# lyclyc52/NeRF_RPN

Measured on AMD Instinct MI355X. Metric: scenes/sec (160^3x4 grids, VGG19-3D+FPN+RPN fwd+bwd), higher is better.
Workload: dtype bf16; 1 GPU; configs[1]: one 160x160x160x4 rgb-sigma grid per GPU, VGG19-EF 3D + FPN + anchor RPN (OBB, 16 GT boxes per scene), fwd+bwd+clip+AdamW, random-init weights; scenes_per_gpu=1, parallelism=dp1, world_size_seen=1, backend=single process

## Files before the change

include/nerfrpn.h:

```cpp
#ifndef NERFRPN_H
#define NERFRPN_H

#include <stddef.h>
#include <stdint.h>

#ifdef __cplusplus
extern "C" {
#endif

typedef void *nrpn_stream_t;

enum nrpn_status {
  NRPN_OK = 0,
  NRPN_ERR_ARG = -1,
  NRPN_ERR_LAUNCH = -2,
  NRPN_ERR_DEVICE = -3
};

enum nrpn_dtype { NRPN_F32 = 0, NRPN_BF16 = 1 };

const char *nrpn_last_error(void);
int nrpn_abi_version(void);
int nrpn_check_device(int ordinal);

// ... 44 lines not shown
                         const int32_t *d_count, int64_t n, int box_dim, int post_top_n, float *out_boxes,
                         float *out_scores, float *out_levels, int32_t *d_out_count, nrpn_stream_t stream);

int nrpn_match_anchors_f32(const int32_t *table, int64_t total_anchors, const float *gt_aabb, int num_gt,
                           float fg_thresh, float bg_thresh, const float *h_ori_size3, float *labels,
                           int32_t *matched, float *workspace, nrpn_stream_t stream);
int nrpn_obb_to_aabb_f32(const float *obb, float *aabb, int64_t n, nrpn_stream_t stream);

size_t nrpn_sample_workspace_bytes(void);
int nrpn_sample_pos_neg(const float *labels, int64_t total, int max_pos, int batch, int64_t seed, void *workspace, int64_t *out_pos,
                        int64_t *out_neg, int32_t *counts, nrpn_stream_t stream);
int nrpn_rpn_sampled_loss_f32(const float *logits, const float *deltas, int dw, const float *targets,
                              const int64_t *pos, int64_t npos, const int64_t *neg, int64_t nneg, float beta,
                              float *loss2, float *g_logits, float *g_deltas, nrpn_stream_t stream);

enum { NRPN_CONV_BIAS = 1, NRPN_CONV_RELU = 2, NRPN_CONV_OUT_F32 = 4,
       NRPN_CONV_DEBUG_ALIAS_TAPS = 256, NRPN_CONV_DEBUG_NO_SYNC = 512,
       NRPN_CONV_DEBUG_STAGGER = 1024,
       NRPN_CONV_DEBUG_VARIANT = 0x3000 };
int nrpn_pack_conv_weight(const float *w_ref, int cout, int cin, int taps, int dtype, void *wp_fwd, void *wp_dgrad,
                          int rows_total, int row_offset, nrpn_stream_t stream);
int nrpn_unpack_conv_wgrad(const float *gw_packed, int cout, int cin, int taps, int rows_total, int row_offset,
                           float *gw_ref, int accumulate, int slices, nrpn_stream_t stream);
size_t nrpn_conv3d_fwd_workspace_bytes(int n, int gx, int gy, int gz, int cin, int cout, int ksize, int dtype);
int nrpn_conv3d_fwd(const void *x, const void *wp, const float *bias, void *y, int n, int gx, int gy, int gz, int cin,
                    int cout, int wrows, int ksize, int dtype, int flags, void *workspace, const void *relu_mask,
                    nrpn_stream_t stream);
enum { NRPN_TILE_AUTO = 0, NRPN_TILE_128 = 128, NRPN_TILE_256X128_WS = 256, NRPN_TILE_256X256 = 512, NRPN_TILE_256X256_W4 = 1024,
       NRPN_TILE_HALO = 2048  };
typedef struct nrpn_conv_opts {
  int32_t size;
  int32_t tile;
  int32_t lds_dma;
  int32_t kstep_bytes;
  int32_t stagger;
  int32_t big_split;
  int32_t debug;
  int32_t halo_pairing;
  const float *scale;
  const void *relu_mask;
  float *stats;
} nrpn_conv_opts;
int nrpn_conv3d_fwd_ex(const void *x, const void *wp, const float *bias, void *y, int n, int gx, int gy, int gz, int cin,
                       int cout, int wrows, int ksize, int dtype, int flags, void *workspace, const nrpn_conv_opts *opts,
                       nrpn_stream_t stream);
size_t nrpn_conv3d_fwd_workspace_bytes_ex(int n, int gx, int gy, int gz, int cin, int cout, int ksize, int dtype,
                                          const nrpn_conv_opts *opts);
int nrpn_conv3d_fwd_plan_ex(int n, int gx, int gy, int gz, int cin, int cout, int ksize, int dtype, const nrpn_conv_opts *opts);
int nrpn_conv3d_fwd_stats_rows_ex(int n, int gx, int gy, int gz, int cin, int cout, int ksize, int dtype, const nrpn_conv_opts *opts);
size_t nrpn_conv3d_wgrad_workspace_bytes(int n, int gx, int gy, int gz, int cin, int cout, int wrows, int ksize, int dtype);
int nrpn_conv3d_wgrad_slices(int n, int gx, int gy, int gz, int cin, int cout, int wrows, int ksize, int dtype);
enum { NRPN_WGRAD_ACC_BIAS = 1, NRPN_WGRAD_MASK_READY = 2,
       NRPN_WGRAD_DEFER_BIAS = 4  };
int nrpn_conv3d_wgrad(const void *x, const void *dy, float *gw_packed, float *gbias, int n, int gx, int gy, int gz,
                      int cin, int cout, int wrows, int ksize, int dtype, int accumulate_bias, void *workspace,
                      nrpn_stream_t stream);
int nrpn_conv3d_fwd_ragged(const void *x, const void *wp, const float *bias, void *y, int nseg, const int32_t *dims, int cin,
                           int cout, int wrows, int ksize, int dtype, int flags, void *workspace, nrpn_stream_t stream);
int nrpn_conv3d_wgrad_ragged(const void *x, const void *dy, float *gw_packed, float *gbias, int nseg, const int32_t *dims,
                             int cin, int cout, int wrows, int ksize, int dtype, int accumulate_bias, void *workspace,
                             nrpn_stream_t stream);
size_t nrpn_cone_workspace_bytes(int64_t total_voxels);
int nrpn_cone_build(const int64_t *pos, const int64_t *neg, const int32_t *counts, int n_scenes, int64_t pos_stride, int64_t neg_stride,
                    int nlevels, const int64_t *level_anchor_off, int num_anchors, const int32_t *dims, int depth, uint32_t *lists,
                    int64_t cap, int32_t *counts_out, void *workspace, nrpn_stream_t stream);
size_t nrpn_conv3d_fwd_rows_workspace_bytes(int64_t nrows, int cin, int cout, int ksize, int dtype);
int nrpn_conv3d_fwd_rows(const void *x, const void *wp, const float *bias, void *y, const uint32_t *rows, int64_t nrows, int nseg,
                         const int32_t *dims, int cin, int cout, int wrows, int ksize, int dtype, int flags, const void *relu_mask,
                         void *workspace, nrpn_stream_t stream);
int nrpn_conv3d_wgrad_rows(const void *x, const void *dy, float *gw_packed, float *gbias, const uint32_t *rows, int64_t nrows, int nseg,
                           const int32_t *dims, int cin, int cout, int wrows, int ksize, int dtype, int accumulate_bias, void *workspace,
                           nrpn_stream_t stream);
int nrpn_conv3d_fwd_plan(int n, int gx, int gy, int gz, int cin, int cout, int ksize, int dtype);
int nrpn_conv3d_fwd_stats_rows(int n, int gx, int gy, int gz, int cin, int cout, int ksize, int dtype);
int nrpn_conv3d_fwd_stats(const void *x, const void *wp, const float *bias, void *y, int n, int gx, int gy, int gz, int cin,
                          int cout, int wrows, int ksize, int dtype, int flags, float *stats, nrpn_stream_t stream);
int nrpn_bn_stats_finalize(const float *partials, int nparts, int64_t rows, int c, float *mean, float *var, float *running_mean,
                           float *running_var, float momentum, nrpn_stream_t stream);
int nrpn_conv3d_wgrad_plan(int n, int gx, int gy, int gz, int cin, int cout, int wrows, int ksize, int dtype);
int nrpn_stem_kpad(int dtype);
int nrpn_pack_stem_weight(const float *w_ref, int cout, int dtype, void *wp, nrpn_stream_t stream);
int nrpn_stem_wgrad_slices(int n, int gx, int gy, int gz, int cout, int stride, int dtype);
int64_t nrpn_stem_wgrad_slice_floats(int n, int gx, int gy, int gz, int cout, int stride, int dtype);
int nrpn_unpack_stem_wgrad(const float *gw_packed, int cout, int dtype, float *gw_ref, int accumulate, int slices,
                           int64_t slice_floats, nrpn_stream_t stream);
int nrpn_conv3d_stem_fwd(const void *x, const void *wp, const float *bias, void *y, int n, int gx, int gy, int gz,
                         int cout, int stride, int dtype, int flags, nrpn_stream_t stream);
int nrpn_stem_halo_supported(int gz, int cout, int stride, int dtype);
int nrpn_stem_halo_kpad(void);
int nrpn_pack_stem_weight_halo(const float *w_ref, int cout, void *wp, nrpn_stream_t stream);
int nrpn_conv3d_stem_fwd_halo(const void *x, const void *wp, const float *bias, const float *scale, void *y, int n, int gx, int gy,
                              int gz, int cout, int flags, nrpn_stream_t stream);
int nrpn_conv3d_stem_fwd_ex(const void *x, const void *wp, const float *bias, void *y, int n, int gx, int gy, int gz,
                            int cout, int stride, int dtype, int flags, const nrpn_conv_opts *opts, nrpn_stream_t stream);
size_t nrpn_stem_wgrad_workspace_bytes(int n, int gx, int gy, int gz, int cout, int stride, int dtype);
int nrpn_conv3d_stem_wgrad(const void *x, const void *dy, float *gw_packed, float *gbias, int n, int gx, int gy, int gz,
                           int cout, int stride, int dtype, int accumulate_bias, void *workspace, nrpn_stream_t stream);

size_t nrpn_bn_workspace_bytes(int64_t rows, int c);
int nrpn_bn_stats(const void *x, int64_t rows, int c, int dtype, float *mean, float *var, float *running_mean,
                  float *running_var, float momentum, void *workspace, nrpn_stream_t stream);
int nrpn_bn_apply(const void *x, void *y, int64_t rows, int c, int dtype, const float *mean, const float *var,
                  const float *gamma, const float *beta, float eps, int relu, nrpn_stream_t stream);
int nrpn_bn_backward(const void *x, const void *y, const void *dy, void *dx, int64_t rows, int c, int dtype,
                     const float *mean, const float *var, const float *gamma, const float *beta, float eps, int relu,
                     float *dgamma, float *dbeta, float *acc_dgamma, float *acc_dbeta, void *workspace, nrpn_stream_t stream);
int nrpn_relu_backward(const void *y, const void *dy, void *dx, int64_t count, int dtype, nrpn_stream_t stream);
int nrpn_pool_out_size(int in, int k, int s, int p, int ceil_mode);
int nrpn_maxpool3d_fwd(const void *x, void *y, int8_t *argmax, int n, int gx, int gy, int gz, int c, int k, int s,
                       int p, int ceil_mode, int dtype, nrpn_stream_t stream);
int nrpn_maxpool3d_bwd(const void *dy, const int8_t *argmax, void *dx, int n, int gx, int gy, int gz, int c, int k,
                       int s, int p, int ceil_mode, int dtype, nrpn_stream_t stream);
int nrpn_upsample_add_fwd(void *fine, const void *coarse, int n, int fx, int fy, int fz, int cx, int cy, int cz, int c,
                          int dtype, nrpn_stream_t stream);
int nrpn_upsample_add_bwd(const void *dfine, void *dcoarse, int n, int fx, int fy, int fz, int cx, int cy, int cz,
                          int c, int dtype, int accumulate, nrpn_stream_t stream);
int nrpn_subsample3d(const void *src, void *dst, int n, int gx, int gy, int gz, int c, int stride, int backward, int dtype,
                     nrpn_stream_t stream);
int nrpn_add_relu(const void *a, const void *b, void *y, int64_t count, int relu, int dtype, nrpn_stream_t stream);
int nrpn_ingest_rgbsigma(const void *src, int src_is_u8, void *dst, int64_t voxels, int alpha_mode, int dtype, nrpn_stream_t stream);
int nrpn_ingest_augment(const void *src, int src_is_u8, void *dst, int w, int l, int h, int alpha_mode, int dtype, int rot90,
                        int z_up, int flip0, int flip1, const float *h_xform, nrpn_stream_t stream);
int nrpn_ncdhw_to_ndhwc(const float *src, void *dst, int n, int c, int64_t voxels, int dtype, nrpn_stream_t stream);
int nrpn_ndhwc_to_ncdhw(const void *src, float *dst, int n, int c, int64_t voxels, int dtype, nrpn_stream_t stream);
int nrpn_cast(const void *src, void *dst, int64_t count, int src_dtype, int dst_dtype, nrpn_stream_t stream);
size_t nrpn_column_sum_workspace_bytes(int64_t rows, int c);
int nrpn_column_sum_f32(const float *x, int64_t rows, int c, float *out, int accumulate, void *workspace, nrpn_stream_t stream);
int nrpn_split_bf16x3(const float *src, int64_t rows, int c, void *interleaved, int ipattern, void *planes, int nplanes, int ppattern,
                      nrpn_stream_t stream);

int nrpn_patchify(const void *x, void *y, int n, int gx, int gy, int gz, int patch, int dtype, nrpn_stream_t stream);
int nrpn_layernorm_fwd(const void *x, void *y, const float *gamma, const float *beta, float *mean, float *rstd, int64_t rows,
                       int c, float eps, int dtype, nrpn_stream_t stream);
size_t nrpn_layernorm_workspace_bytes(int64_t rows, int c);
int nrpn_layernorm_bwd(const void *x, const void *dy, void *dx, const float *gamma, const float *mean, const float *rstd,
                       float *dgamma, float *dbeta, int64_t rows, int c, int dtype, int accumulate_params, void *workspace,
                       nrpn_stream_t stream);
int nrpn_gelu(const void *x, const void *dy, void *out, int64_t count, int backward, int dtype, nrpn_stream_t stream);
int nrpn_scale_add(const void *a, const void *b, const float *scale, void *y, int n, int64_t per_sample, int dtype,
                   nrpn_stream_t stream);
int nrpn_patch_merge(const void *src, void *dst, int n, int gx, int gy, int gz, int c, int backward, int dtype,
                     nrpn_stream_t stream);
int nrpn_window_attn_fwd(const void *qkv, const float *qkv_bias, const float *bias_table, const int32_t *rel_index, void *out,
                         int n, int gx, int gy, int gz, int c, int heads, int shift, int dtype, nrpn_stream_t stream);
size_t nrpn_window_attn_bwd_workspace_bytes(int n, int gx, int gy, int gz, int heads);
int nrpn_window_attn_bwd(const void *qkv, const float *qkv_bias, const float *bias_table, const int32_t *rel_index,
                         const void *dout, void *dqkv, float *dtable, float *dbias_pad, int n, int gx, int gy, int gz, int c,
                         int heads, int shift, int dtype, int accumulate_table, void *workspace, nrpn_stream_t stream);

size_t nrpn_groupnorm_workspace_bytes(int n, int c, int groups);
int nrpn_groupnorm_fwd(const void *x, void *y, const float *gamma, const float *beta, float *mean, float *rstd, int n,
                       int64_t rows, int c, int groups, float eps, int relu, int dtype, void *workspace, nrpn_stream_t stream);
int nrpn_groupnorm_bwd(const void *x, const void *y, const void *dy, void *dx, const float *gamma, const float *mean,
                       const float *rstd, float *dgamma, float *dbeta, int n, int64_t rows, int c, int groups, int relu, int dtype,
                       int accumulate_params, void *workspace, nrpn_stream_t stream);
int nrpn_fcos_reduce_floats(void);
int nrpn_fcos_head_out_f32(const float *cls_out, const float *box_out, int wrows, const float *scale, float stride_mul,
                           int norm_reg, int reg_dim, int ctr_on_reg, int64_t rows, float *logits, float *reg, float *ctr,
                           nrpn_stream_t stream);
int nrpn_fcos_head_out_bwd_f32(const float *box_out, int wrows, const float *scale, float stride_mul, int norm_reg, int reg_dim,
                               int ctr_on_reg, int64_t rows, const float *d_logits, const float *d_reg, const float *d_ctr,
                               float *d_cls_out, float *d_box_out, float *d_scale, nrpn_stream_t stream);
int nrpn_fcos_gt_summary_f32(const float *gt, int count, int width, float *summary, nrpn_stream_t stream);
int nrpn_fcos_targets_f32(const float *summary, const int32_t *gt_offsets, int n, int levels, const int32_t *dims,
                          const int32_t *strides, const float *ori_sizes, float radius, int norm_reg, int reg_dim, int8_t *labels,
                          float *reg_targets, int32_t *num_pos, nrpn_stream_t stream);
// ... 148 lines not shown
```

include/nerfrpn_tools.h:

```cpp
#ifndef NERFRPN_TOOLS_H
#define NERFRPN_TOOLS_H
#include "nerfrpn.h"

#ifdef __cplusplus
extern "C" {
#endif

int nrpn_set_conv_kstep_bytes(int kb);
int nrpn_set_conv_lds_dma(int on);
int nrpn_set_conv_tile_m(int bm);
int nrpn_set_conv_halo_auto(int on);
int nrpn_set_conv_halo_pairing(int mode);
int nrpn_set_conv_stagger(int on);
int nrpn_set_conv_big_split(int on);
int nrpn_set_wgrad_big_tile(int on);
int nrpn_set_wgrad_pack2(int on);
int nrpn_set_sumsq_form(int form, int grid);
int nrpn_set_wgrad_transpose_read(int on);
int nrpn_set_rows_big_tile(int on);
int nrpn_set_rows_tail_split(int on);
int nrpn_set_bn_fast(int on);
int nrpn_set_bn_reduce_v8(int on);
int nrpn_set_pool_fast(int on);
int nrpn_set_gn_fast(int on);
int64_t nrpn_fastdiv_host(int64_t n, int64_t d);
int nrpn_set_window_attn_mfma(int on);

#ifdef __cplusplus
}
#endif
#endif
```

nerf_rpn_amd/csrc/conv3d.hip:

```cpp
#include "conv_common.cuh"
#include "conv_plan.h"

#ifndef NRPN_HALO_PAIRING_DEFAULT
#define NRPN_HALO_PAIRING_DEFAULT 2
#endif

template <typename T, int BN, int MODE, bool OUTF32, int KB, bool GLDS, int BM = 128, bool ROWS = false>
__global__ void __launch_bounds__(256, BM == 128 ? 2 : 1) conv_igemm_kernel(const ConvArgs p) {
  constexpr int WAVES_N = (BN == 128) ? 2 : 1;
  constexpr int TM = BM / (32 * (4 / WAVES_N));
  constexpr int TN = 2;
  constexpr int KE = KB / (int)sizeof(T);
  constexpr int PPR = KB / 16;
  constexpr int RSTEP = 256 / PPR;
  constexpr int A_RPT = BM / RSTEP;
  constexpr int B_RPT = BN / RSTEP;
  constexpr int SWZ_SH = (KB == 64) ? 2 : 1;
  constexpr int A_BYTES = BM * KB, B_BYTES = BN * KB;
  extern __shared__ __attribute__((aligned(16))) char lds[];

  const int tid = threadIdx.x, lane = tid & 63, wave = tid >> 6;
  const int wm = wave / WAVES_N, wn = wave % WAVES_N;
  const unsigned ntiles = (p.Cout + BN - 1) / BN;
  const unsigned tiles = (unsigned)((p.M + BM - 1) / BM) * ntiles;
// ... 2480 lines not shown
  return wgrad_plan(conv_shape(n, gx, gy, gz, cin, cout, wrows, ksize, dtype), cin, 0, wg_knobs());
}
extern "C" size_t nrpn_conv3d_wgrad_bias_offset(int n, int gx, int gy, int gz, int ksize) {
  return wgrad_mask_bytes((long long)n * gx * gy * gz, ksize == 3 ? 27 : 1);
}
extern "C" size_t nrpn_conv3d_wgrad_workspace_bytes(int n, int gx, int gy, int gz, int cin, int cout, int wrows, int ksize, int dtype) {
  const WgPlan pl = wgrad_query(n, gx, gy, gz, cin, cout, wrows, ksize, dtype);
  return pl.bias_off + pl.bias_bytes;
}
extern "C" int nrpn_conv3d_wgrad_plan(int n, int gx, int gy, int gz, int cin, int cout, int wrows, int ksize, int dtype) {
  return wgrad_query(n, gx, gy, gz, cin, cout, wrows, ksize, dtype).big ? 1 : 0;
}
extern "C" int nrpn_conv3d_wgrad_slices(int n, int gx, int gy, int gz, int cin, int cout, int wrows, int ksize, int dtype) {
  return wgrad_query(n, gx, gy, gz, cin, cout, wrows, ksize, dtype).ksplit;
}

static int conv3d_wgrad_impl(const void *x, const void *dy, float *gw_packed, float *gbias, long long M, int gx, int gy, int gz,
                             const Segs *segs, int cin, int cout, int wrows, int ksize, int dtype, int accumulate_bias, void *workspace,
                             nrpn_stream_t stream, const unsigned *rows = nullptr, long long total_voxels = 0) {
  NRPN_REQUIRE(ksize == 1 || ksize == 3, "conv3d_wgrad: ksize must be 1 or 3 (got %d)", ksize);
  NRPN_REQUIRE(dtype == NRPN_F32 || dtype == NRPN_BF16, "conv3d_wgrad: bad dtype %d", dtype);
  const int es = dtype == NRPN_F32 ? 4 : 2;
  NRPN_REQUIRE((cin * es) % 16 == 0 && (cout * es) % 16 == 0, "conv3d_wgrad: channel rows must be 16-byte multiples (Cin=%d Cout=%d)", cin, cout);
  NRPN_REQUIRE(x && dy && gw_packed && wrows >= cout, "conv3d_wgrad: bad args");
  WgradArgs a{};
  a.x = x; a.dy = dy; a.gw = gw_packed;
  a.M = M;
  a.X = gx; a.Y = gy; a.Z = gz; a.OX = gx; a.OY = gy; a.OZ = gz;
  if (segs) a.segs = *segs;
  a.Cin = cin; a.Cout = cout; a.wrows = wrows; a.taps = ksize == 3 ? 27 : 1; a.stride = 1; a.kpad = 0;
  hipStream_t st = as_stream(stream);
  NRPN_REQUIRE(workspace, "conv3d_wgrad: needs its workspace (nrpn_conv3d_wgrad_workspace_bytes)");
  const long long span = rows ? total_voxels : a.M;
  NRPN_REQUIRE(span * cin * es < (1ll << 31) && span * cout * es < (1ll << 31) && a.M * 8 < (1ll << 31), "conv3d_wgrad: tensors must stay below 2 GiB");
  a.x_bytes = (unsigned)(span * cin * es); a.dy_bytes = (unsigned)(span * cout * es);
  a.rows = rows;
  a.vmask = reinterpret_cast<const unsigned *>(workspace);
  const bool mask_ready = (accumulate_bias & NRPN_WGRAD_MASK_READY) != 0;
  const bool defer_bias = (accumulate_bias & NRPN_WGRAD_DEFER_BIAS) != 0;
  accumulate_bias &= NRPN_WGRAD_ACC_BIAS;
  if (ksize == 3 && !mask_ready && !rows)
    hipLaunchKernelGGL(tap_mask_kernel, dim3((unsigned)cdiv64(a.M, 256)), dim3(256), 0, st, reinterpret_cast<unsigned *>(workspace), a.M, gx, gy, gz,
                       a.segs);
  const WgPlan pl = wgrad_plan(ConvShape{M, 0, gx, gy, gz, cin, cout, wrows, a.taps, es, segs != nullptr}, cin, 0, wg_knobs(), rows != nullptr);
  float *bias_part = reinterpret_cast<float *>(reinterpret_cast<char *>(workspace) + pl.bias_off);
  a.gbias = gbias ? bias_part : nullptr;
  a.slice_stride = (long long)a.taps * wrows * cin;
  const int rc = (dtype == NRPN_F32) ? launch_wgrad<float, 0>(a, pl, st) : launch_wgrad<bf16s, 0>(a, pl, st);
  if (rc || !gbias || defer_bias) return rc;
  hipLaunchKernelGGL(bias_finalize_kernel, dim3((unsigned)((cout + 255) / 256)), dim3(256), 0, st, bias_part, pl.ksplit, wrows, cout, gbias,
                     accumulate_bias);
  NRPN_LAUNCH_CHECK("bias_finalize");
  return NRPN_OK;
}

extern "C" int nrpn_conv3d_wgrad(const void *x, const void *dy, float *gw_packed, float *gbias, int n, int gx, int gy, int gz, int cin,
                                 int cout, int wrows, int ksize, int dtype, int accumulate_bias, void *workspace, nrpn_stream_t stream) {
  NRPN_REQUIRE(n > 0 && gx > 0 && gy > 0 && gz > 0, "conv3d_wgrad: bad sizes");
  return conv3d_wgrad_impl(x, dy, gw_packed, gbias, (long long)n * gx * gy * gz, gx, gy, gz, nullptr, cin, cout, wrows, ksize, dtype,
                           accumulate_bias, workspace, stream);
}

extern "C" int nrpn_conv3d_wgrad_ragged(const void *x, const void *dy, float *gw_packed, float *gbias, int nseg, const int32_t *dims,
                                        int cin, int cout, int wrows, int ksize, int dtype, int accumulate_bias, void *workspace,
                                        nrpn_stream_t stream) {
  Segs sg{};
  long long M = 0;
  if (int rc = fill_segs(sg, nseg, dims, M)) return rc;
  return conv3d_wgrad_impl(x, dy, gw_packed, gbias, M, 1, 1, 1, &sg, cin, cout, wrows, ksize, dtype, accumulate_bias, workspace, stream);
}

extern "C" int nrpn_conv3d_wgrad_rows(const void *x, const void *dy, float *gw_packed, float *gbias, const uint32_t *rows, int64_t nrows,
                                      int nseg, const int32_t *dims, int cin, int cout, int wrows, int ksize, int dtype, int accumulate_bias,
                                      void *workspace, nrpn_stream_t stream) {
  NRPN_REQUIRE(rows && nrows > 0, "conv3d_wgrad_rows: empty row list (the caller zero-fills the gradient instead)");
  Segs sg{};
  long long total = 0;
  if (int rc = fill_segs(sg, nseg, dims, total)) return rc;
  NRPN_REQUIRE(workspace, "conv3d_wgrad_rows: needs a workspace (>= 256 bytes; slices * wrows floats with a bias gradient)");
  return conv3d_wgrad_impl(x, dy, gw_packed, gbias, nrows, 1, 1, 1, &sg, cin, cout, wrows, ksize, dtype, accumulate_bias | NRPN_WGRAD_MASK_READY,
                           workspace, stream, rows, total);
}

static long long stem_out_voxels(int n, int gx, int gy, int gz, int stride) {
  return (long long)n * ((gx - 1) / stride + 1) * ((gy - 1) / stride + 1) * ((gz - 1) / stride + 1);
}

static StemWgPlan stem_wgrad_query(int n, int gx, int gy, int gz, int cout, int stride, int dtype) {
  return stem_wgrad_plan(stem_out_voxels(n, gx, gy, gz, stride), gz, cout, stride, dtype == NRPN_F32 ? 4 : 2, wg_knobs());
}
extern "C" int nrpn_stem_wgrad_slices(int n, int gx, int gy, int gz, int cout, int stride, int dtype) {
  return stem_wgrad_query(n, gx, gy, gz, cout, stride, dtype).slices;
}
extern "C" int64_t nrpn_stem_wgrad_slice_floats(int n, int gx, int gy, int gz, int cout, int stride, int dtype) {
  return stem_wgrad_query(n, gx, gy, gz, cout, stride, dtype).slice_floats;
}
extern "C" size_t nrpn_stem_wgrad_workspace_bytes(int n, int gx, int gy, int gz, int cout, int stride, int dtype) {
  return stem_wgrad_query(n, gx, gy, gz, cout, stride, dtype).ws_bytes;
}

extern "C" int nrpn_conv3d_stem_wgrad(const void *x, const void *dy, float *gw_packed, float *gbias, int n, int gx, int gy, int gz,
                                      int cout, int stride, int dtype, int accumulate_bias, void *workspace, nrpn_stream_t stream) {
  NRPN_REQUIRE(stride == 1 || stride == 2, "stem wgrad: stride must be 1 or 2 (got %d)", stride);
  NRPN_REQUIRE(dtype == NRPN_F32 || dtype == NRPN_BF16, "stem wgrad: bad dtype %d", dtype);
  const int es = dtype == NRPN_F32 ? 4 : 2;
  NRPN_REQUIRE((cout * es) % 16 == 0, "stem wgrad: Cout row must be a 16-byte multiple");
  NRPN_REQUIRE(x && dy && gw_packed, "stem wgrad: null pointer");
  WgradArgs a{};
  a.x = x; a.dy = dy; a.gw = gw_packed;
  a.X = gx; a.Y = gy; a.Z = gz;
  a.OX = (gx - 1) / stride + 1; a.OY = (gy - 1) / stride + 1; a.OZ = (gz - 1) / stride + 1;
  a.M = (long long)n * a.OX * a.OY * a.OZ;
  a.Cin = 4; a.Cout = cout; a.wrows = cout; a.taps = 343; a.stride = stride;
  a.kpad = stem_kpad(es);
  hipStream_t st = as_stream(stream);
  {
    const long long xb = (long long)n * gx * gy * gz * 4 * es, db = a.M * cout * es;
    NRPN_REQUIRE(xb < (1ll << 31) && db < (1ll << 31), "stem wgrad: tensors must stay below 2 GiB");
    a.x_bytes = (unsigned)xb; a.dy_bytes = (unsigned)db; a.vmask = nullptr;
  }
  NRPN_REQUIRE(!gbias || workspace, "stem wgrad: the bias gradient needs the workspace (nrpn_stem_wgrad_workspace_bytes)");
  const StemWgPlan pl = stem_wgrad_plan(a.M, gz, cout, stride, es, wg_knobs());
  if (pl.zrow) {
    StemZrArgs z{};
    z.x = x; z.dy = dy; z.gw = gw_packed; z.gbias = gbias ? reinterpret_cast<float *>(workspace) : nullptr;
    z.M = a.M; z.X = gx; z.Y = gy; z.Z = gz; z.OX = a.OX; z.OY = a.OY; z.OZ = a.OZ;
    z.slices = pl.slices;
    z.x_bytes = a.x_bytes; z.dy_bytes = a.dy_bytes;
    const dim3 grid((unsigned)(7 * z.slices));
    if (dtype == NRPN_F32) {
      constexpr size_t lds_ = 2 * (size_t)(ZrCfg<float>::KV * ZrCfg<float>::RSA + 7 * ZrCfg<float>::KV * ZrCfg<float>::RSB);
      NRPN_LDS((stem_wgrad_zrow_kernel<float>), (int)lds_);
      hipLaunchKernelGGL(stem_wgrad_zrow_kernel<float>, grid, dim3(256), lds_, st, z);
    } else {
      constexpr size_t lds_ = 2 * (size_t)(ZrCfg<bf16s>::KV * ZrCfg<bf16s>::RSA + 7 * ZrCfg<bf16s>::KV * ZrCfg<bf16s>::RSB);
      NRPN_LDS((stem_wgrad_zrow_kernel<bf16s>), (int)lds_);
      hipLaunchKernelGGL(stem_wgrad_zrow_kernel<bf16s>, grid, dim3(256), lds_, st, z);
    }
    NRPN_LAUNCH_CHECK("stem_wgrad_zrow");
    if (!gbias) return NRPN_OK;
    hipLaunchKernelGGL(bias_finalize_kernel, dim3(1), dim3(256), 0, st, z.gbias, z.slices, cout, cout, gbias, accumulate_bias);
    NRPN_LAUNCH_CHECK("bias_finalize");
    return NRPN_OK;
  }
  a.gbias = gbias ? reinterpret_cast<float *>(workspace) : nullptr;
  a.slice_stride = pl.slice_floats;
  const int rc = (dtype == NRPN_F32) ? launch_wgrad<float, 1>(a, pl.gemm, st) : launch_wgrad<bf16s, 1>(a, pl.gemm, st);
  if (rc || !gbias) return rc;
  hipLaunchKernelGGL(bias_finalize_kernel, dim3((unsigned)((cout + 255) / 256)), dim3(256), 0, st, a.gbias, pl.slices, cout, cout, gbias,
                     accumulate_bias);
  NRPN_LAUNCH_CHECK("bias_finalize");
  return NRPN_OK;
}

template <typename T>
__global__ void pack_weight_kernel(const float *__restrict__ w, int cout, int cin, int taps, T *__restrict__ fwd, T *__restrict__ dgrad,
                                   int rows_total, int row_offset) {
  const long long i = (long long)blockIdx.x * blockDim.x + threadIdx.x;
  const long long total = (long long)cout * cin * taps;
  if (i >= total) return;
  const int t = (int)(i % taps);
  const int c = (int)((i / taps) % cin);
  const int o = (int)(i / ((long long)taps * cin));
  const float v = w[i];
  if (fwd) elem<T>::st(fwd + ((long long)t * rows_total + row_offset + o) * cin + c, v);
  if (dgrad) elem<T>::st(dgrad + ((long long)(taps - 1 - t) * cin + c) * rows_total + row_offset + o, v);
}

extern "C" int nrpn_pack_conv_weight(const float *w_ref, int cout, int cin, int taps, int dtype, void *wp_fwd, void *wp_dgrad,
                                     int rows_total, int row_offset, nrpn_stream_t stream) {
  NRPN_REQUIRE(w_ref && (wp_fwd || wp_dgrad) && cout > 0 && cin > 0 && taps > 0 && row_offset >= 0 && row_offset + cout <= rows_total,
               "pack_conv_weight: bad args");
  const long long total = (long long)cout * cin * taps;
  dim3 grid((unsigned)cdiv64(total, 256));
  if (dtype == NRPN_F32)
    hipLaunchKernelGGL(pack_weight_kernel<float>, grid, dim3(256), 0, as_stream(stream), w_ref, cout, cin, taps, (float *)wp_fwd,
                       (float *)wp_dgrad, rows_total, row_offset);
  else
    hipLaunchKernelGGL(pack_weight_kernel<bf16s>, grid, dim3(256), 0, as_stream(stream), w_ref, cout, cin, taps, (bf16s *)wp_fwd,
                       (bf16s *)wp_dgrad, rows_total, row_offset);
  NRPN_LAUNCH_CHECK("pack_conv_weight");
  return NRPN_OK;
}

__global__ void __launch_bounds__(256) unpack_wgrad_kernel(const float *__restrict__ gp, int cout, int cin, int taps, int rows_total,
                                                           int row_offset, float *__restrict__ gw, int accumulate, int slices,
                                                           long long slice_stride) {
  __shared__ float tile[27][65];
  const int o = blockIdx.y, c0 = blockIdx.x * 64;
  for (int i = threadIdx.x; i < taps * 64; i += 256) {
    const int t = i / 64, c = i % 64;
    float v = 0.f;
    if (c0 + c < cin) {
      const float *src = gp + ((long long)t * rows_total + row_offset + o) * cin + c0 + c;
      for (int s = 0; s < slices; ++s) v += src[s * slice_stride];
    }
    tile[t][c] = v;
  }
  __syncthreads();
  const int ncol = min(64, cin - c0);
  float *dst = gw + ((long long)o * cin + c0) * taps;
  for (int i = threadIdx.x; i < ncol * taps; i += 256) {
    const float v = tile[i % taps][i / taps];
    dst[i] = accumulate ? dst[i] + v : v;
  }
}

extern "C" int nrpn_unpack_conv_wgrad(const float *gw_packed, int cout, int cin, int taps, int rows_total, int row_offset, float *gw_ref,
                                      int accumulate, int slices, nrpn_stream_t stream) {
  NRPN_REQUIRE(gw_packed && gw_ref && cout > 0 && cin > 0 && taps > 0 && taps <= 27 && slices > 0 && row_offset + cout <= rows_total,
               "unpack_conv_wgrad: bad args");
  hipLaunchKernelGGL(unpack_wgrad_kernel, dim3((unsigned)((cin + 63) / 64), (unsigned)cout), dim3(256), 0, as_stream(stream), gw_packed, cout,
                     cin, taps, rows_total, row_offset, gw_ref, accumulate, slices, (long long)taps * rows_total * cin);
// ... 51 lines not shown
```

Before: 113.7 scenes/sec.

## Add ring-buffered stem weight-gradient kernel that reuses input rows across output rows

Adds a new kernel for the stride-2 7x7x7 stem weight gradient. It keeps a 16-slot LDS ring of padded input z-rows so that consecutive output rows reuse 5 of the 7 y-rows already loaded, and only the 2 new rows are fetched per step. It also prefetches dy tiles several rows ahead with LDS DMA and computes on MFMA using transposed LDS reads in inline asm. The kernel is enabled by default when the shape fits, replacing the zrow kernel. The risk is lower occupancy from the larger LDS footprint and added complexity in hand-written waitcnt and barrier handling.

```diff
diff --git a/include/nerfrpn.h b/include/nerfrpn.h
--- a/include/nerfrpn.h
+++ b/include/nerfrpn.h
@@ -150,6 +150,7 @@
 int nrpn_pack_stem_weight(const float *w_ref, int cout, int dtype, void *wp, nrpn_stream_t stream);
 int nrpn_stem_wgrad_slices(int n, int gx, int gy, int gz, int cout, int stride, int dtype);
 int64_t nrpn_stem_wgrad_slice_floats(int n, int gx, int gy, int gz, int cout, int stride, int dtype);
+int nrpn_stem_wgrad_form(int n, int gx, int gy, int gz, int cout, int stride, int dtype);
 int nrpn_unpack_stem_wgrad(const float *gw_packed, int cout, int dtype, float *gw_ref, int accumulate, int slices,
                            int64_t slice_floats, nrpn_stream_t stream);
 int nrpn_conv3d_stem_fwd(const void *x, const void *wp, const float *bias, void *y, int n, int gx, int gy, int gz,
diff --git a/include/nerfrpn_tools.h b/include/nerfrpn_tools.h
--- a/include/nerfrpn_tools.h
+++ b/include/nerfrpn_tools.h
@@ -24,6 +24,7 @@
 int nrpn_set_pool_fast(int on);
 int nrpn_set_gn_fast(int on);
 int64_t nrpn_fastdiv_host(int64_t n, int64_t d);
+int nrpn_set_stem_wgrad_ring(int on);
 int nrpn_set_window_attn_mfma(int on);
 
 #ifdef __cplusplus
diff --git a/nerf_rpn_amd/csrc/conv3d.hip b/nerf_rpn_amd/csrc/conv3d.hip
--- a/nerf_rpn_amd/csrc/conv3d.hip
+++ b/nerf_rpn_amd/csrc/conv3d.hip
@@ -2586,6 +2586,8 @@
                            workspace, stream, rows, total);
 }
 
+#include "stem_wgrad.h"
+
 static long long stem_out_voxels(int n, int gx, int gy, int gz, int stride) {
   return (long long)n * ((gx - 1) / stride + 1) * ((gy - 1) / stride + 1) * ((gz - 1) / stride + 1);
 }
@@ -2632,7 +2634,9 @@
     z.slices = pl.slices;
     z.x_bytes = a.x_bytes; z.dy_bytes = a.dy_bytes;
     const dim3 grid((unsigned)(7 * z.slices));
-    if (dtype == NRPN_F32) {
+    if (stem_wgrad_ring_applies(gz, es)) {
+      if (int rc = stem_wgrad_ring_launch(x, dy, gw_packed, z.gbias, z.M, gx, gy, gz, z.slices, z.x_bytes, z.dy_bytes, dtype, st)) return rc;
+    } else if (dtype == NRPN_F32) {
       constexpr size_t lds_ = 2 * (size_t)(ZrCfg<float>::KV * ZrCfg<float>::RSA + 7 * ZrCfg<float>::KV * ZrCfg<float>::RSB);
       NRPN_LDS((stem_wgrad_zrow_kernel<float>), (int)lds_);
       hipLaunchKernelGGL(stem_wgrad_zrow_kernel<float>, grid, dim3(256), lds_, st, z);
diff --git a/nerf_rpn_amd/csrc/stem_wgrad.h b/nerf_rpn_amd/csrc/stem_wgrad.h
--- /dev/null
+++ b/nerf_rpn_amd/csrc/stem_wgrad.h
@@ -0,0 +1,6 @@
+#pragma once
+#include <hip/hip_runtime.h>
+
+bool stem_wgrad_ring_applies(int gz, int elem_bytes);
+int stem_wgrad_ring_launch(const void *x, const void *dy, float *gw, float *gbias_part, long long M, int gx, int gy, int gz, int slices,
+                           unsigned x_bytes, unsigned dy_bytes, int dtype, hipStream_t st);
diff --git a/nerf_rpn_amd/csrc/stem_wgrad.hip b/nerf_rpn_amd/csrc/stem_wgrad.hip
--- /dev/null
+++ b/nerf_rpn_amd/csrc/stem_wgrad.hip
@@ -0,0 +1,352 @@
+#include "conv_common.cuh"
+#include "conv_plan.h"
+#include "stem_wgrad.h"
+
+template <typename T> struct RingCfg;
+template <> struct RingCfg<bf16s> { static constexpr int KV = 64, RSA = 64 * 2, KSUB = 16, ZPP = 2, VP = 16; };
+template <> struct RingCfg<float> { static constexpr int KV = 32, RSA = 64 * 4, KSUB = 8, ZPP = 1, VP = 32; };
+constexpr int kSlots = 16;
+
+template <int RS> __device__ __forceinline__ int ring_swz(int row) { return RS >= 256 ? (row & 3) << 2 : ((row >> 1) & 1) << 2; }
+template <int RS> __device__ __forceinline__ int ring_off(int row, int byte_in_row) {
+  return row * RS + ((((byte_in_row >> 4) ^ ring_swz<RS>(row))) << 4) + (byte_in_row & 15);
+}
+__device__ __forceinline__ f4 tr_pair(const char *a0, int second) {
+  const s4v lo = __builtin_amdgcn_ds_read_tr16_b64_v4i16((s4v __attribute__((address_space(3))) *)(a0));
+  const s4v hi = __builtin_amdgcn_ds_read_tr16_b64_v4i16((s4v __attribute__((address_space(3))) *)(a0 + second));
+  typedef __attribute__((ext_vector_type(2))) long long l2v;
+  l2v r = {__builtin_bit_cast(long long, lo), __builtin_bit_cast(long long, hi)};
+  return __builtin_bit_cast(f4, r);
+}
+template <typename T, int RS> __device__ __forceinline__ f4 dy_frag(const char *tile, int ctile0, int kbase, int lane) {
+  const int h = lane >> 5;
+  if (sizeof(T) == 4) {
+    const int c = ctile0 + (lane & 31);
+    f4 v;
+#pragma unroll
+    for (int q = 0; q < 4; ++q) v[q] = *reinterpret_cast<const float *>(tile + ring_off<RS>(kbase + 4 * h + q, c * 4));
+    return v;
+  } else {
+    const int p = lane & 15;
+    const int cbase = ctile0 + 16 * ((lane >> 4) & 1);
+    const int row = kbase + 8 * h + (p >> 2);
+    return tr_pair(tile + ring_off<RS>(row, (cbase + 4 * (p & 3)) * 2), 4 * RS);
+  }
+}
+template <typename T, int VP> __device__ __forceinline__ f4 row_frag(const char *row, int kbase, int lane) {
+  const int h = lane >> 5;
+  if (sizeof(T) == 4) {
+    f4 v;
+#pragma unroll
+    for (int q = 0; q < 4; ++q) v[q] = *reinterpret_cast<const float *>(row + (kbase + 4 * h + q) * VP + (lane & 31) * 4);
+    return v;
+  } else {
+    const int p = lane & 15;
+    return tr_pair(row + (kbase + 8 * h + (p >> 2)) * VP + (16 * ((lane >> 4) & 1) + 4 * (p & 3)) * 2, 4 * VP);
+  }
+}
+
+typedef __attribute__((ext_vector_type(2))) int i2v;
+__device__ __forceinline__ f4 pair_f4(i2v lo, i2v hi) {
+  typedef __attribute__((ext_vector_type(4))) int i4v;
+  const i4v r = {lo[0], lo[1], hi[0], hi[1]};
+  return __builtin_bit_cast(f4, r);
+}
+__device__ __forceinline__ void read_group2(unsigned a0, unsigned a1, unsigned b0, unsigned b1, f4 &af0, f4 &af1, f4 &bf0, f4 &bf1) {
+  i2v r0, r1, r2, r3, r4, r5, r6, r7;
+  asm volatile("ds_read_b64_tr_b16 %0, %8\n\t"
+               "ds_read_b64_tr_b16 %1, %8 offset:512\n\t"
+               "ds_read_b64_tr_b16 %2, %9\n\t"
+               "ds_read_b64_tr_b16 %3, %9 offset:512\n\t"
+               "ds_read_b64_tr_b16 %4, %10\n\t"
+               "ds_read_b64_tr_b16 %5, %10 offset:64\n\t"
+               "ds_read_b64_tr_b16 %6, %11\n\t"
+               "ds_read_b64_tr_b16 %7, %11 offset:64\n\t"
+               "s_waitcnt lgkmcnt(0)"
+               : "=&v"(r0), "=&v"(r1), "=&v"(r2), "=&v"(r3), "=&v"(r4), "=&v"(r5), "=&v"(r6), "=&v"(r7)
+               : "v"(a0), "v"(a1), "v"(b0), "v"(b1)
+               : "memory");
+  af0 = pair_f4(r0, r1); af1 = pair_f4(r2, r3); bf0 = pair_f4(r4, r5); bf1 = pair_f4(r6, r7);
+}
+__device__ __forceinline__ void read_group1(unsigned a0, unsigned a1, unsigned b0, f4 &af0, f4 &af1, f4 &bf0) {
+  i2v r0, r1, r2, r3, r4, r5;
+  asm volatile("ds_read_b64_tr_b16 %0, %6\n\t"
+               "ds_read_b64_tr_b16 %1, %6 offset:512\n\t"
+               "ds_read_b64_tr_b16 %2, %7\n\t"
+               "ds_read_b64_tr_b16 %3, %7 offset:512\n\t"
+               "ds_read_b64_tr_b16 %4, %8\n\t"
+               "ds_read_b64_tr_b16 %5, %8 offset:64\n\t"
+               "s_waitcnt lgkmcnt(0)"
+               : "=&v"(r0), "=&v"(r1), "=&v"(r2), "=&v"(r3), "=&v"(r4), "=&v"(r5)
+               : "v"(a0), "v"(a1), "v"(b0)
+               : "memory");
+  af0 = pair_f4(r0, r1); af1 = pair_f4(r2, r3); bf0 = pair_f4(r4, r5);
+}
+__device__ __forceinline__ f4 lds_read16(unsigned addr) {
+  f4 v;
+  asm volatile("ds_read_b128 %0, %1\n\ts_waitcnt lgkmcnt(0)" : "=&v"(v) : "v"(addr) : "memory");
+  return v;
+}
+
+__device__ __forceinline__ void ring_wait_vm(int n) {
+#define RING_VM(k) case k: asm volatile("s_waitcnt vmcnt(" #k ")" ::: "memory"); break;
+  switch (n) {
+    RING_VM(1) RING_VM(2) RING_VM(3) RING_VM(4) RING_VM(5) RING_VM(6) RING_VM(7) RING_VM(8) RING_VM(9) RING_VM(10) RING_VM(11) RING_VM(12)
+    RING_VM(13) RING_VM(14) RING_VM(15) RING_VM(16) RING_VM(17) RING_VM(18) RING_VM(19) RING_VM(20) RING_VM(21) RING_VM(22) RING_VM(23) RING_VM(24)
+    default: asm volatile("s_waitcnt vmcnt(0)" ::: "memory"); break;
+  }
+#undef RING_VM
+}
+template <typename T> __device__ __forceinline__ void ring_barrier() {
+  if (sizeof(T) == 2) asm volatile("s_barrier" ::: "memory");
+  else __syncthreads();
+}
+
+struct StemRingArgs {
+  const void *x, *dy;
+  float *gw;
+  float *gbias;
+  long long M;
+  int X, Y, Z, OX, OY, OZ;
+  int slices;
+  unsigned x_bytes, dy_bytes;
+  int na;
+  int np;
+  int rpb;
+  int depth;
+};
+
+template <typename T>
+__global__ void __launch_bounds__(256, 2) stem_wgrad_ring_kernel(const StemRingArgs p) {
+  constexpr int KV = RingCfg<T>::KV, RSA = RingCfg<T>::RSA, KSUB = RingCfg<T>::KSUB, ZPP = RingCfg<T>::ZPP, VP = RingCfg<T>::VP;
+  constexpr int COUT = 64, APR = RSA / 16, EPP = 16 / (int)sizeof(T);
+  extern __shared__ __attribute__((aligned(16))) char lds[];
+
+  const int tid = threadIdx.x, lane = tid & 63, wave = tid >> 6;
+  const int wave_u = __builtin_amdgcn_readfirstlane(wave);
+  const int dx = blockIdx.x % 7, slice = blockIdx.x / 7;
+  const long long chunks = (p.M + KV - 1) / KV;
+  const long long per = (chunks + p.slices - 1) / p.slices;
+  const long long c_begin = slice * per, c_end = min(chunks, c_begin + per);
+  const int v0 = (int)(c_begin * KV), v1 = (int)min(p.M, c_end * KV);
+  const int r0 = v0 / p.OZ, r1 = (v1 - 1) / p.OZ;
+
+  const __amdgpu_buffer_rsrc_t xr = make_rsrc(p.x, p.x_bytes), dyr = make_rsrc(p.dy, p.dy_bytes);
+  const int a_bytes = p.na * 4096;
+  char *ring = lds + (p.depth + 1) * a_bytes;
+  const int a_k0 = tid / APR, a_slot = (tid % APR) ^ ring_swz<RSA>(tid / APR);
+
+  auto issue = [&](int r, int j, int oy, int n, int ox, int bufi) {
+    char *A = lds + bufi * a_bytes;
+    const int vrow = r * p.OZ;
+    for (int i = 0; i < p.na; ++i) {
+      const int k = a_k0 + (256 / APR) * i, v = vrow + k;
+      const bool ok = k < p.OZ && v >= v0 && v < v1;
+      lds_dma16(dyr, A + (64 * wave_u + 256 * i) * 16, ok ? (unsigned)v * (unsigned)RSA + (unsigned)(a_slot * 16) : kOOB);
+    }
+    const int ix = 2 * ox - 3 + dx;
+    const bool xok = (unsigned)ix < (unsigned)p.X;
+    const int plane = (n * p.X + ix) * p.Y;
+    int c = 0;
+    for (int t = j == 0 ? 0 : 5; t < 7; ++t) {
+      const int iy = 2 * oy - 3 + t;
+      const bool rok = xok && (unsigned)iy < (unsigned)p.Y;
+      const int rowvox = (plane + iy) * p.Z;
+      char *dst = ring + ((2 * j + t) & (kSlots - 1)) * p.rpb;
+      for (int s = 0; s < p.np; s += 64, ++c) {
+        if ((c & 3) != wave_u) continue;
+        const int start = min(s, max(p.np - 64, 0));
+        const int pc = start + lane;
+        const int zp = pc * ZPP - 4;
+        const bool ok = rok && zp >= 0 && zp + ZPP <= p.Z;
+        lds_dma16(xr, dst + start * 16, ok ? (unsigned)(rowvox + zp) * (unsigned)(4 * sizeof(T)) : kOOB);
+      }
+    }
+  };
+  const int row_cnt = p.na + ((2 * ((p.np + 63) / 64) - wave_u + 3) >> 2);
+
+  const int t0 = wave_u, t1 = wave_u + 4;
+  const bool two = t1 < 7;
+  f16v acc[2][2];
+#pragma unroll
+  for (int i = 0; i < 2; ++i)
+#pragma unroll
+    for (int j = 0; j < 2; ++j)
+#pragma unroll
+      for (int r = 0; r < 16; ++r) acc[i][j][r] = 0.f;
+  const bool do_bias = p.gbias != nullptr && dx == 0;
+  float bias_acc[EPP];
+#pragma unroll
+  for (int e = 0; e < EPP; ++e) bias_acc[e] = 0.f;
+
+  const unsigned lds_base = (unsigned)(size_t)(__attribute__((address_space(3))) char *)lds, ring_base = lds_base + (unsigned)((p.depth + 1) * a_bytes);
+  const int f_p = lane & 15, f_row = 8 * (lane >> 5) + (f_p >> 2), f_c = 16 * ((lane >> 4) & 1) + 4 * (f_p & 3);
+  const unsigned fa0 = (unsigned)ring_off<RSA>(f_row, f_c * 2), fa1 = (unsigned)ring_off<RSA>(f_row, (32 + f_c) * 2);
+  const unsigned fb = (unsigned)(f_row * VP + f_c * 2);
+
+  const int D = p.depth, nb = D + 1;
+  int r = r0, oy, ox, n, gi = 0, gc = 0;
+  {
+    const int q = r0 / p.OY;
+    oy = r0 - q * p.OY; n = q / p.OX; ox = q - n * p.OX;
+  }
+  while (r <= r1) {
+    const int len = min(p.OY - oy, r1 - r + 1);
+    for (int j = 0; j < min(D, len); ++j) {
+      issue(r + j, j, oy + j, n, ox, gi);
+      gi = gi + 1 == nb ? 0 : gi + 1;
+    }
+    for (int j = 0; j < len; ++j) {
+      ring_wait_vm(sizeof(T) == 2 ? row_cnt * min(D - 1, len - 1 - j) : 0);
+      ring_barrier<T>();
+      if (j + D < len) {
+        issue(r + j + D, j + D, oy + j + D, n, ox, gi);
+        gi = gi + 1 == nb ? 0 : gi + 1;
+      }
+      const int sb = 2 * j;
+      if constexpr (sizeof(T) == 2) {
+        const unsigned a = lds_base + (unsigned)(gc * a_bytes);
+        if (do_bias) {
+          for (int i = 0; i < p.na; ++i) {
+            typedef __attribute__((ext_vector_type(8))) unsigned short u8v;
+            const u8v hh = __builtin_bit_cast(u8v, lds_read16(a + (unsigned)((tid + 256 * i) * 16)));
+#pragma unroll
+            for (int e = 0; e < 8; ++e) bias_acc[e] += bf16_bits_to_f32(hh[e]);
+          }
+        }
+        unsigned a0 = a + fa0, a1 = a + fa1;
+        unsigned b0 = ring_base + (unsigned)(((sb + t0) & (kSlots - 1)) * p.rpb) + fb;
+        unsigned b1 = ring_base + (unsigned)(((sb + t1) & (kSlots - 1)) * p.rpb) + fb;
+        if (two) {
+          for (int kb = 0; kb < p.OZ; kb += KSUB) {
+            f4 af[2], bf0, bf1;
+            read_group2(a0, a1, b0, b1, af[0], af[1], bf0, bf1);
+#pragma unroll
+            for (int i = 0; i < 2; ++i) {
+              Mma<T>::run(acc[i][0], af[i], bf0);
+              Mma<T>::run(acc[i][1], af[i], bf1);
+            }
+            a0 += KSUB * RSA; a1 += KSUB * RSA; b0 += KSUB * VP; b1 += KSUB * VP;
+          }
+        } else {
+          for (int kb = 0; kb < p.OZ; kb += KSUB) {
+            f4 af[2], bf0;
+            read_group1(a0, a1, b0, af[0], af[1], bf0);
+#pragma unroll
+            for (int i = 0; i < 2; ++i) Mma<T>::run(acc[i][0], af[i], bf0);
+            a0 += KSUB * RSA; a1 += KSUB * RSA; b0 += KSUB * VP;
+          }
+        }
+      } else {
+        const char *A = lds + gc * a_bytes;
+        const char *B0 = ring + ((sb + t0) & (kSlots - 1)) * p.rpb;
+        const char *B1 = ring + ((sb + t1) & (kSlots - 1)) * p.rpb;
+        if (do_bias) {
+          for (int i = 0; i < p.na; ++i) {
+            const f4 v = *reinterpret_cast<const f4 *>(A + (tid + 256 * i) * 16);
+#pragma unroll
+            for (int e = 0; e < 4; ++e) bias_acc[e] += v[e];
+          }
+        }
+        for (int kb = 0; kb < p.OZ; kb += KSUB) {
+          f4 af[2], bf0, bf1 = zero4();
+          af[0] = dy_frag<T, RSA>(A, 0, kb, lane);
+          af[1] = dy_frag<T, RSA>(A, 32, kb, lane);
+          bf0 = row_frag<T, VP>(B0, kb, lane);
+          if (two) bf1 = row_frag<T, VP>(B1, kb, lane);
+#pragma unroll
+          for (int i = 0; i < 2; ++i) {
+            Mma<T>::run(acc[i][0], af[i], bf0);
+            if (two) Mma<T>::run(acc[i][1], af[i], bf1);
+          }
+        }
+      }
+      gc = gc + 1 == nb ? 0 : gc + 1;
+    }
+    ring_barrier<T>();
+    r += len;
+    oy += len;
+    if (oy == p.OY) {
+      oy = 0;
+      if (++ox == p.OX) { ox = 0; ++n; }
+    }
+  }
+
+  if (do_bias) {
+    constexpr int NRG = 256 / APR;
+    float *red = reinterpret_cast<float *>(lds);
+#pragma unroll
+    for (int e = 0; e < EPP; ++e) red[tid * EPP + e] = bias_acc[e];
+    __syncthreads();
+    if (tid < COUT) {
+      const int g = tid / EPP, e = tid % EPP;
+      float sum = 0.f;
+      for (int rg = 0; rg < NRG; ++rg) sum += red[(rg * APR + (g ^ ring_swz<RSA>(rg))) * EPP + e];
+      p.gbias[(long long)slice * COUT + tid] = sum;
+    }
+  }
+  const int fr = lane & 31;
+#pragma unroll
+  for (int j = 0; j < 2; ++j) {
+    if (j == 1 && !two) continue;
+    const int tap = dx * 7 + (j == 0 ? t0 : t1);
+    float *dst = p.gw + ((long long)slice * 49 + tap) * COUT * 32;
+#pragma unroll
+    for (int i = 0; i < 2; ++i)
+#pragma unroll
+      for (int r = 0; r < 16; ++r) dst[(i * 32 + frag_row(r, lane)) * 32 + fr] = acc[i][j][r];
+  }
+}
+
+static std::atomic<int> g_stem_ring{1};
+
+struct RingShape {
+  bool ok;
+  int na, np, rpb, depth;
+  size_t lds;
+};
+static RingShape ring_shape(int gz, int elem_bytes) {
+  RingShape s{};
+  const int oz = gz / 2, apr = elem_bytes == 2 ? 8 : 16, ksub = elem_bytes == 2 ? 16 : 8;
+  s.na = (oz * apr + 255) / 256;
+  s.np = (gz + 6) * 4 * elem_bytes / 16;
+  s.rpb = (s.np > 64 ? s.np : 64) * 16;
+  for (s.depth = elem_bytes == 2 ? 3 : 1; s.depth >= 1; --s.depth) {
+    s.lds = (size_t)(s.depth + 1) * s.na * 4096 + (size_t)kSlots * s.rpb;
+    if (s.lds <= 80 * 1024) break;
+  }
+  s.ok = oz > 0 && oz % ksub == 0 && s.depth >= 1;
+  return s;
+}
+
+extern "C" int nrpn_set_stem_wgrad_ring(int on) { g_stem_ring = on ? 1 : 0; return NRPN_OK; }
+
+bool stem_wgrad_ring_applies(int gz, int elem_bytes) { return g_stem_ring.load() != 0 && ring_shape(gz, elem_bytes).ok; }
+
+extern "C" int nrpn_stem_wgrad_form(int n, int gx, int gy, int gz, int cout, int stride, int dtype) {
+  const int es = dtype == NRPN_F32 ? 4 : 2;
+  const long long M = (long long)n * ((gx - 1) / stride + 1) * ((gy - 1) / stride + 1) * ((gz - 1) / stride + 1);
+  if (!stem_wgrad_plan(M, gz, cout, stride, es, WgKnobs{1, 1, 1}).zrow) return 0;
+  return stem_wgrad_ring_applies(gz, es) ? 2 : 1;
+}
+
+int stem_wgrad_ring_launch(const void *x, const void *dy, float *gw, float *gbias_part, long long M, int gx, int gy, int gz, int slices,
+                           unsigned x_bytes, unsigned dy_bytes, int dtype, hipStream_t st) {
+  const RingShape s = ring_shape(gz, dtype == NRPN_F32 ? 4 : 2);
+  NRPN_REQUIRE(s.ok, "stem wgrad ring: Z = %d is not a ring shape", gz);
+  StemRingArgs a{};
+  a.x = x; a.dy = dy; a.gw = gw; a.gbias = gbias_part;
+  a.M = M; a.X = gx; a.Y = gy; a.Z = gz; a.OX = (gx - 1) / 2 + 1; a.OY = (gy - 1) / 2 + 1; a.OZ = gz / 2;
+  a.slices = slices; a.x_bytes = x_bytes; a.dy_bytes = dy_bytes;
+  a.na = s.na; a.np = s.np; a.rpb = s.rpb; a.depth = s.depth;
+  const dim3 grid((unsigned)(7 * slices));
+  if (dtype == NRPN_F32) {
+    NRPN_LDS((stem_wgrad_ring_kernel<float>), (int)s.lds);
+    hipLaunchKernelGGL(stem_wgrad_ring_kernel<float>, grid, dim3(256), s.lds, st, a);
+  } else {
+    NRPN_LDS((stem_wgrad_ring_kernel<bf16s>), (int)s.lds);
+    hipLaunchKernelGGL(stem_wgrad_ring_kernel<bf16s>, grid, dim3(256), s.lds, st, a);
+  }
+  NRPN_LAUNCH_CHECK("stem_wgrad_ring");
+  return NRPN_OK;
+}
```

Result: no change. 113.9 scenes/sec (median of 5 runs) (+0.2%).
